# szpajder/dumpvdl2

Hardware: AMD Instinct MI355X
Metric: IQ MS/s demodulated end-to-end (higher is better)
Workload: dtype f32

## Files before the change

dumpvdl2_amd/csrc/debug_hooks.inc:

```

static bool hip_ok(hipError_t e) { return e == hipSuccess; }
template<typename T> static bool dbg_up(const DevBuf<T> &d, const void *src, size_t bytes) { return hip_ok(hipMemcpy(d, src, bytes, hipMemcpyHostToDevice)); }
template<typename T> static bool dbg_up(const DevBuf<T> &d, const void *src) { return dbg_up(d, src, d.bytes()); }
template<typename T> static bool dbg_fill(const DevBuf<T> &d, int v) { return hip_ok(hipMemset(d, v, d.bytes())); }
template<typename T> static bool dbg_down(void *dst, const DevBuf<T> &d, size_t bytes) { return hip_ok(hipMemcpy(dst, d, bytes, hipMemcpyDeviceToHost)); }
template<typename T> static bool dbg_down(void *dst, const DevBuf<T> &d) { return dbg_down(dst, d, d.bytes()); }
static bool dbg_tables(const DevBuf<Tables> &d) { auto tab = std::make_unique<Tables>(); build_tables(*tab); return dbg_up(d, tab.get()); }

template<int K> static int prof_read(const void *symbol, unsigned long long *out, int reset) {
	unsigned long long h[64][K];
	if(hipMemcpyFromSymbol(h, symbol, sizeof h) != hipSuccess) return -3;
	for(int k = 0; k < K; k++) { out[k] = 0; for(int s = 0; s < 64; s++) out[k] += h[s][k]; }
	if(reset) { memset(h, 0, sizeof h); if(hipMemcpyToSymbol(symbol, h, sizeof h) != hipSuccess) return -3; }
	return 0;
}

extern "C" {

int vdl2hip_debug_live_resources(long long out[3]) {
	if(!out) return VDL2HIP_E_INVAL;
	for(int i = 0; i < 3; i++) out[i] = hostmem::g_live[i].load();
	return VDL2HIP_OK;
}

// ... 41 lines not shown
	DevBuf<ScanReq> d_sq, d_rt; DevBuf<uint32_t> d_n;
	if(!hip_ok(d_sq.alloc(count)) || !hip_ok(d_n.alloc(2)) || !hip_ok(d_rt.alloc(kRetryScans))) return VDL2HIP_E_NOMEM;
	uint32_t before[8] = {0}, after[8] = {0};
	const uint32_t nn[2] = { count, 0u };
	Event e0, e1;
	if(!hip_ok(e0.ensure()) || !hip_ok(e1.ensure()) || !dbg_up(d_sq, h.data()) || !dbg_up(d_n, nn) || !dbg_down(before, c->d_refstats, sizeof before)) return VDL2HIP_E_DEVICE;
	RefChan *ref = c->d_ref[(c->feed_no - 1) % kSlots];
	launch_scans(c, c->streams.front, ref, 0xfffeu, d_sq, nullptr, d_n, count, c->k_total, with_retry ? d_rt.get() : nullptr, d_n + 1, e0, e1);
	if(!hip_ok(hipStreamSynchronize(c->streams.front)) || !dbg_down(after, c->d_refstats, sizeof after)) return VDL2HIP_E_DEVICE;
	if(ms) { float t = 0.f; (void)hipEventElapsedTime(&t, e0, e1); *ms = t; }
	return (int)(after[0] - before[0]);
}
int vdl2hip_debug_exact_window(vdl2hip_ctx *c, uint32_t chan, int64_t n_lo, int64_t n_hi) { return vdl2hip_debug_exact_window_many(c, chan, n_lo, n_hi, 1, 0, nullptr); }

int vdl2hip_debug_u8_levels(float out[512]) {
	DevBuf<float> d;
	if(!hip_ok(d.alloc(512))) return VDL2HIP_E_NOMEM;
	hipLaunchKernelGGL(k_u8_level_probe, dim3(1), dim3(256), 0, 0, d);
	return dbg_down(out, d) ? VDL2HIP_OK : VDL2HIP_E_DEVICE;
}

int vdl2hip_debug_s8_levels(float out[512]) {
	DevBuf<float> d;
	if(!hip_ok(d.alloc(512))) return VDL2HIP_E_NOMEM;
	hipLaunchKernelGGL(k_s8_level_probe, dim3(1), dim3(256), 0, 0, d);
	return dbg_down(out, d) ? VDL2HIP_OK : VDL2HIP_E_DEVICE;
}

int vdl2hip_debug_dpp_probe(const float in[64], float out[256]) {
	DevBuf<float> d_in, d_out;
	if(!hip_ok(d_in.alloc(64)) || !hip_ok(d_out.alloc(256))) return VDL2HIP_E_NOMEM;
	if(!dbg_up(d_in, in)) return VDL2HIP_E_DEVICE;
	hipLaunchKernelGGL(k_dpp_probe, dim3(1), dim3(64), 0, 0, (const float *)d_in, d_out);
	return dbg_down(out, d_out) ? VDL2HIP_OK : VDL2HIP_E_DEVICE;
}

int vdl2hip_debug_core_probe(int kind, const void *in, size_t n, void *out) {
	if(kind < 0 || kind >= PROBE_KINDS || !in || !out || n == 0 || n > (size_t)1 << 26) return VDL2HIP_E_INVAL;
	DevBuf<float> d_in, d_out; DevBuf<Tables> d_tab;
	if(!hip_ok(d_in.alloc(n * (size_t)core_probe_in_words(kind))) || !hip_ok(d_out.alloc(n * (size_t)core_probe_out_words(kind))) || !hip_ok(d_tab.alloc(1))) return VDL2HIP_E_NOMEM;
	if(!dbg_tables(d_tab) || !dbg_up(d_in, in) || !dbg_fill(d_out, 0)) return VDL2HIP_E_DEVICE;
	hipLaunchKernelGGL(k_core_probe, dim3((unsigned)((n + 255) / 256)), dim3(256), 0, 0, kind, (const float *)d_in, (uint32_t)n, d_out, (const Tables *)d_tab);
	return hip_ok(hipGetLastError()) && dbg_down(out, d_out) ? VDL2HIP_OK : VDL2HIP_E_DEVICE;
}

int vdl2hip_debug_burst_probe(int kind, const void *in, size_t n, unsigned grid, void *out, const uint32_t *freq, uint32_t nchan, const float *y, uint32_t ring_len,
		uint32_t cap_frames, uint32_t cap_pool, uint32_t guard_frames, uint32_t guard_pool, void *frames, uint8_t *pool, void *ctl, unsigned long long *cnt) {
	if(kind < 0 || kind >= BPROBE_KINDS || !in || n == 0 || n > (size_t)1 << 20 || grid == 0 || grid > 1024) return VDL2HIP_E_INVAL;
	const uint32_t nwaves = grid * (uint32_t)kBurstWaves;
	const bool burst = kind == BPROBE_BURST;
	size_t nin = 0, nout = 0;
	if(kind == BPROBE_WAVE) { nin = n * 64 * 4; nout = n * (size_t)kBProbeWaveOut * 4; }
	else if(kind == BPROBE_RS) {
		nin = n * (size_t)kBProbeRsStride; nout = n * (size_t)kBProbeRsStride + n * 4;
		for(size_t i = 0; i < n; i++) { const uint8_t np = ((const uint8_t *)in)[i * kBProbeRsStride + kRsN]; if(np > kRsPar || (np & 1)) return VDL2HIP_E_INVAL; }
	} else {
		nin = n * sizeof(Burst);
		if(!freq || nchan == 0 || !y || ring_len < 64 || (ring_len & (ring_len - 1)) || ring_len > 1u << 20 || !frames || !pool || !ctl || !cnt) return VDL2HIP_E_INVAL;
		if(cap_frames > 1u << 20 || cap_pool > 1u << 26 || guard_frames > 1u << 16 || guard_pool > 1u << 20 || n * (size_t)ring_len > (size_t)1 << 26) return VDL2HIP_E_INVAL;
		for(size_t i = 0; i < n; i++) {
			const Burst &b = ((const Burst *)in)[i];
			if(b.chan < 0 || (uint32_t)b.chan >= nchan || b.nsym < 1 || b.nsym > kMaxSyms || b.tl_bits == 0 || b.tl_bits > kMaxTl || b.t_first < 0 || b.prev_n < -2) return VDL2HIP_E_INVAL;
		}
	}
	if(!burst && !out) return VDL2HIP_E_INVAL;
	const size_t nfr = (size_t)cap_frames + guard_frames, npool = (size_t)cap_pool + guard_pool;
// ... 393 lines not shown
```

dumpvdl2_amd/csrc/kernels.h:

```cpp
#pragma once
#include <hip/hip_runtime.h>
#include <type_traits>
#include "vdl2_core.h"
#include "design.h"

#ifndef VDL2_K1_UNROLL
#define VDL2_K1_UNROLL 5
#endif

#ifndef VDL2_K1_WAVES_PER_EU
#define VDL2_K1_WAVES_PER_EU 3
#endif

namespace vdl2 {

constexpr int kK1Unroll = VDL2_K1_UNROLL;
typedef float v2f __attribute__((ext_vector_type(2)));
typedef float v4f __attribute__((ext_vector_type(4)));

#ifndef VDL2_REF_PRIO
#define VDL2_REF_PRIO 3
#endif
#ifndef VDL2_K1_PRIO
#define VDL2_K1_PRIO 0
// ... 239 lines not shown
	const int c = (chan + (int)blockIdx.x) % nchan;
	const int64_t off = stride * (int64_t)blockIdx.x;
	ChanView v{ ref->y + (size_t)c * ref->cap, nullptr, nullptr, ref->mask, ref, c, 0xffffu };
	const bool ok = ref_exact_window(v, n_lo + off, n_hi + off, scratch, REF_CANDIDATE);
	if(threadIdx.x == 0) out[blockIdx.x] = ok ? 1 : 0;
}

VDL2_HD bool ref_window_done(const ChanView &v, int64_t n_lo, int64_t n_hi) {
#if VDL2_DEVICE_PASS
	return ref_window_done_dev(v, n_lo, n_hi);
#else
	(void)v; (void)n_lo; (void)n_hi;
	return false;
#endif
}
VDL2_HD __attribute__((always_inline)) bool ref_exact_window(const ChanView &v, int64_t n_lo, int64_t n_hi, void *scratch, int kind) {
#if VDL2_DEVICE_PASS
	(void)scratch;
	return ref_exact_window_dev(v, n_lo, n_hi, kind);
#else
	(void)v; (void)n_lo; (void)n_hi; (void)scratch; (void)kind;
	return false;
#endif
}

struct K1Consts {
	float g0[kMaxOversample], g1[kMaxOversample];
	float P[4], c0, c1, c2, pad_;
	float Q[6][4];
	float Pp[kRunMax + 1][4];
	float cP[kRunMax][2];
};

inline K1Consts make_k1_consts(const BlockForm &bf) {
	K1Consts k{};
	for(int i = 0; i < kMaxOversample; i++) { k.g0[i] = bf.g0[i]; k.g1[i] = bf.g1[i]; }
	for(int i = 0; i < 4; i++) k.P[i] = bf.P[i];
	k.c0 = bf.c0; k.c1 = bf.c1; k.c2 = bf.c2;
	for(int d = 0; d < 6; d++) for(int i = 0; i < 4; i++) k.Q[d][i] = bf.Q[d][i];
	for(int r = 0; r <= kRunMax; r++) for(int i = 0; i < 4; i++) k.Pp[r][i] = bf.Ppow[r][i];
	for(int r = 0; r < kRunMax; r++) { k.cP[r][0] = bf.cP[r][0]; k.cP[r][1] = bf.cP[r][1]; }
	return k;
}

struct K1Args {
	const void *in;
	const void *carry;
	uint32_t ncarry;
	uint64_t nlogical;
	uint64_t n0;
	int64_t  k0;
	int64_t  D;
	int32_t  fmt, nchan, os, nseg, gy;
	int32_t  seg0, seg1;
	const uint32_t *dphi;
	const Lut4 *lut;
	K1Consts bf;
	cf32 *y;
	float4 *seg_end;
	const float4 *qpow;
	int32_t  tiles;
	int32_t  fuse;
	const float4 *carry_in;
	float4 *carry_out;
	const BlockForm *bfd;
	unsigned long long *seg_pub;
	uint32_t epoch;
	uint32_t pub_epoch;
	uint32_t spin_limit;
	uint32_t *sync_timeouts;
	uint32_t cap, mask, nseg_cap;
// ... 27 lines not shown
__device__ __forceinline__ float dpp_row_shr(float v, int d) {
	const int x = __builtin_bit_cast(int, v);
	int r;
	switch(d) {
		case 0: r = __builtin_amdgcn_update_dpp(0, x, 0x111, 0xf, 0xf, true); break;
		case 1: r = __builtin_amdgcn_update_dpp(0, x, 0x112, 0xf, 0xf, true); break;
		case 2: r = __builtin_amdgcn_update_dpp(0, x, 0x114, 0xf, 0xf, true); break;
		default: r = __builtin_amdgcn_update_dpp(0, x, 0x118, 0xf, 0xf, true); break;
	}
	return __builtin_bit_cast(float, r);
}
template<int CTRL, int ROWS>
__device__ __forceinline__ float dpp_bcast(float v) {
	return __builtin_bit_cast(float, __builtin_amdgcn_update_dpp(0, __builtin_bit_cast(int, v), CTRL, ROWS, 0xf, false));
}
template<int CTRL, int ROWS>
__device__ __forceinline__ float dpp_bcast_keep(float old, float v) {
	return __builtin_bit_cast(float, __builtin_amdgcn_update_dpp(__builtin_bit_cast(int, old), __builtin_bit_cast(int, v), CTRL, ROWS, 0xf, false));
}
__device__ __forceinline__ float dpp_wave_shr1_keep(float lane0, float v) {
	return __builtin_bit_cast(float, __builtin_amdgcn_update_dpp(__builtin_bit_cast(int, lane0), __builtin_bit_cast(int, v), 0x138, 0xf, 0xf, false));
}
__device__ __forceinline__ float dpp_wave_shr1(float v) {
	return __builtin_bit_cast(float, __builtin_amdgcn_update_dpp(0, __builtin_bit_cast(int, v), 0x138, 0xf, 0xf, true));
}

__global__ void k_dpp_probe(const float *in, float *out) {
	const int l = threadIdx.x & 63;
	const float v = in[l];
	out[l] = dpp_row_shr(v, 2);
	out[64 + l] = dpp_bcast<0x142, 0xa>(v);
	out[128 + l] = dpp_bcast<0x143, 0xc>(v);
	out[192 + l] = dpp_wave_shr1(v);
}

#ifndef VDL2_K1_MIN_BLOCKS
#define VDL2_K1_MIN_BLOCKS 6
#endif
#ifndef VDL2_K1_MIN_BLOCKS_CR4
#define VDL2_K1_MIN_BLOCKS_CR4 4
#endif
#ifdef VDL2_K1_PROF
__device__ unsigned long long vdl2_k1_prof[64][16];
#define K1_BEGIN() unsigned k1_t0_ = (unsigned)__builtin_readcyclecounter(), k1_acc_[8] = {0, 0, 0, 0, 0, 0, 0, 0}, k1_tiles_ = 0
#define K1_MARK(k) do { if(__builtin_amdgcn_readfirstlane(threadIdx.x >> 6) == 0) { const unsigned t_ = (unsigned)__builtin_readcyclecounter(); \
	k1_acc_[k] += t_ - k1_t0_; if((k) == 3) k1_tiles_++; k1_t0_ = t_; } } while(0)
#define K1_END() do { if(threadIdx.x == 0) { for(int k_ = 0; k_ < 8; k_++) atomicAdd(&vdl2_k1_prof[blockIdx.x & 63][k_], (unsigned long long)k1_acc_[k_]); \
	atomicAdd(&vdl2_k1_prof[blockIdx.x & 63][8], 1ull); atomicAdd(&vdl2_k1_prof[blockIdx.x & 63][9], (unsigned long long)k1_tiles_); } } while(0)
#else
#define K1_BEGIN() do {} while(0)
#define K1_MARK(k) do {} while(0)
#define K1_END() do {} while(0)
#endif

__device__ __forceinline__ float u8_level(uint32_t i) {
	const float d = (float)i - 127.5f, r = 1.0f / 127.5f;
	const float q = d * r;
	return __builtin_fmaf(__builtin_fmaf(-127.5f, q, d), r, q);
}
__global__ void k_u8_level_probe(float *out) { const uint32_t i = threadIdx.x; out[i] = u8_level(i); out[256 + i] = ((float)i - 127.5f) / 127.5f; }
__device__ __forceinline__ float2 s8_level(uint32_t w) {
	const uint32_t u = w ^ 0x8080u;
	return make_float2(__builtin_fmaf((float)(u & 0xffu), 0.0078125f, -1.0f), __builtin_fmaf((float)((u >> 8) & 0xffu), 0.0078125f, -1.0f));
}
__global__ void k_s8_level_probe(float *out) { const uint32_t i = threadIdx.x; out[i] = i & 1 ? s8_level(i << 8).y : s8_level(i).x; out[256 + i] = (float)(int8_t)i / 128.0f; }

// ... 7 lines not shown
	float *o = out + (size_t)i * core_probe_out_words(kind);
	switch(kind) {
	case PROBE_PHASE: o[0] = phase_of(cf32{x[0], x[1]}); break;
	case PROBE_PHASE_FAST: o[0] = phase_fast(cf32{x[0], x[1]}); break;
	case PROBE_MAG: o[0] = mag_of(cf32{x[0], x[1]}); break;
	case PROBE_METRIC: {
		float ph[kPreamble];
		for(int j = 0; j < kPreamble; j++) ph[j] = x[j];
		sync_metric(ph, *tab, o[0], o[1]);
	} break;
	case PROBE_SCREEN: {
		float ph[kPreamble];
		for(int j = 0; j < kPreamble; j++) ph[j] = x[j];
		o[0] = sync_metric_screen(ph, kPreamble); o[1] = sync_metric_screen(ph, kScreenEarly);
	} break;
	case PROBE_SLICE: {
		int neg = 0;
		const int idx = slice_symbol(x[0], x[1], x[2], neg);
		o[0] = __int_as_float(idx); o[1] = __int_as_float(neg);
	} break;
	case PROBE_VERTEX: o[0] = parabola_vertex(x[0], x[1], x[2]); break;
	case PROBE_PPM: {
		const uint32_t freq = __float_as_uint(x[1]);
		o[0] = ppm_of(x[0], freq); o[1] = ppm_gate_threshold(freq, x[2]);
	} break;
	case PROBE_HEADER: {
		const Geometry g = header_to_geometry(__float_as_uint(x[0]), tab->hdr_H, tab->hdr_fix);
		o[0] = __int_as_float(g.status); o[1] = __uint_as_float(g.syndrome); o[2] = __uint_as_float(g.tl_bits); o[3] = __uint_as_float(g.want_bits);
	} break;
	default: break;
	}
}

template<int OS, int R, int CR, bool U8 = false, bool CF32 = false, bool S8 = false>
__global__ __launch_bounds__(256, (CR >= 4 ? VDL2_K1_MIN_BLOCKS_CR4 : VDL2_K1_MIN_BLOCKS)) void k_chanfir(K1Args a) {
	static_assert(64 * R == kFixW || R == 1, "the fused fix-up assumes the fix window is the segment's first tile");
	static_assert(R >= 1 && R <= 2, "the run's outputs are held in two register pairs");
	__shared__ __align__(16) float4 lut[256];
	__shared__ __align__(16) float4 qpow[64];
	__shared__ __align__(16) float park[4 * 4 * 4 * 4];
	__shared__ int fallback;
	constexpr bool kParkY = OS != 0 && CR >= 4 && R == 2;
	__shared__ __align__(8) float2 ypark[kParkY ? CR * 256 : 1];
	extern __shared__ __align__(16) unsigned char smem[];
	if(VDL2_K1_PRIO) __builtin_amdgcn_s_setprio(VDL2_K1_PRIO);
	const int os = OS ? OS : a.os;
	const int run = R * os;
	float2 *tile = (float2 *)smem;
	const int tid = threadIdx.x;
	K1_BEGIN();

	const int bid = blockIdx.x;
	const int xcd = bid & 7, q = bid >> 3;
	const int gy = q % a.gy;
	const int seg = a.seg0 + (q / a.gy) * 8 + xcd;
	if(seg >= a.seg1) return;

	constexpr bool kPrefetch = OS != 0 && CR >= 4 && (64 * R * OS + 255) / 256 <= 10 && (64 * R * OS) % 256 == 0;
	static_assert(!U8 || kPrefetch, "the unsigned-byte build exists where the tile prefetch does");
	static_assert(!CF32 || !U8, "one format per build");
	static_assert(!S8 || (kPrefetch && !U8 && !CF32), "the signed-byte build exists where the unsigned-byte build does, one format per build");
	constexpr bool kByte = U8 || S8;
	constexpr int kFmt = CF32 ? 2 : S8 ? 3 : U8 ? 0 : 1;
	constexpr int kLoadS8 = S8 ? 2 : (kPrefetch && (OS == 20 || OS == 10)) ? 0 : 1;
	constexpr int kPre = kPrefetch ? (64 * R * OS) / 256 : 1;
	constexpr bool kPipeGather = kPrefetch;
	uint32_t pre[kPre]; bool have_pre = false;
	float2 pre2[CF32 ? kPre : 1];
	#pragma unroll
	for(int k = 0; k < kPre; k++) pre[k] = 0u;
	#pragma unroll
	for(int k = 0; k < (CF32 ? kPre : 1); k++) pre2[k] = make_float2(0.f, 0.f);
	if(kPrefetch) {
		const int64_t s0 = (int64_t)seg * a.tiles * (64 * R * (OS ? OS : 1));
		have_pre = a.fmt == kFmt && s0 >= (int64_t)a.ncarry && s0 + 64 * R * (OS ? OS : 1) <= (int64_t)a.nlogical && (int64_t)seg * a.tiles * (64 * R) < a.D;
		if(have_pre) {
			if constexpr(CF32) {
				const float2 *sn = (const float2 *)a.in + (s0 - a.ncarry);
				#pragma unroll
				for(int k = 0; k < kPre; k++) pre2[k] = sn[tid + 256 * k];
			} else if constexpr(kByte) {
				const uint16_t *sn = (const uint16_t *)a.in + (s0 - a.ncarry);
				#pragma unroll
				for(int k = 0; k < kPre; k++) pre[k] = sn[tid + 256 * k];
			} else {
			const uint32_t *sn = (const uint32_t *)a.in + (s0 - a.ncarry);
			#pragma unroll
			for(int k = 0; k < kPre; k++) pre[k] = sn[tid + 256 * k];
			}
		}
	}
	lut[tid] = ((const float4 *)a.lut)[tid];
	if(tid < 64) qpow[tid] = a.qpow[tid];
	if(tid == 0) fallback = 0;
	const int wave = __builtin_amdgcn_readfirstlane(tid >> 6), lane = tid & 63;
	const int cbase = (gy * 4 + wave) * CR;
	const bool wave_active = cbase < a.nchan;
	const K1Consts &bf = a.bf;
	const int tile_n = 64 * run;
	const int L = 64 * R;

	uint32_t dph[CR];
	float4 *carry = (float4 *)(park + wave * (4 * CR * 4));
	float4 *svp = carry + CR;
	float4 *sendp = svp + CR;
	float4 *tsp = sendp + CR;
#ifdef VDL2_K1_HOLD_IN_MEMORY
	constexpr bool kHoldRegs = !(OS != 0 && CR >= 4);
#else
	constexpr bool kHoldRegs = true;
#endif
	float hold[CR][4];
	#pragma unroll
	for(int c = 0; c < CR; c++) hold[c][0] = hold[c][1] = hold[c][2] = hold[c][3] = 0.f;
	#pragma unroll
	for(int c = 0; c < CR; c++) {
		const int ch = cbase + c < a.nchan ? cbase + c : a.nchan - 1;
		dph[c] = a.dphi[ch];
		if(lane == 0) carry[c] = make_float4(0.f, 0.f, 0.f, 0.f);
	}
	const float P0 = bf.P[0], P1 = bf.P[1], P2 = bf.P[2], P3 = bf.P[3];
	const float c0 = bf.c0, c1 = bf.c1, c2 = bf.c2;

	for(int ts = 0; ts < a.tiles; ts++) {
		const int64_t tix = (int64_t)seg * a.tiles + ts;
		const int64_t kbase = tix * L;
		if(kbase >= a.D) break;
		const int64_t sbase = tix * tile_n;
		K1_MARK(ts ? 4 : 0);
		if(ts) __syncthreads();
		K1_MARK(5);
		const bool fast_now = a.fmt == kFmt && sbase >= (int64_t)a.ncarry && sbase + tile_n <= (int64_t)a.nlogical;
		if(CF32 && kPrefetch && fast_now) {
			const float2 *src = (const float2 *)a.in + (sbase - a.ncarry);
			#pragma unroll
			for(int k = 0; k < kPre; k++) {
				const int t = tid + 256 * k;
				const float2 w = have_pre ? pre2[CF32 ? k : 0] : src[t];
				const int l = t / run, m = t - l * run;
				tile[m * 65 + l] = make_float2(cf32_level(w.x), cf32_level(w.y));
			}
			const int64_t snext = sbase + tile_n;
			have_pre = ts + 1 < a.tiles && (tix + 1) * L < a.D && snext + tile_n <= (int64_t)a.nlogical;
			if(have_pre) {
				const float2 *sn = (const float2 *)a.in + (snext - a.ncarry);
				#pragma unroll
				for(int k = 0; k < kPre; k++) pre2[CF32 ? k : 0] = sn[tid + 256 * k];
			}
		} else if(!CF32 && kPrefetch && kByte && fast_now) {
			const uint16_t *src = (const uint16_t *)a.in + (sbase - a.ncarry);
			#pragma unroll
			for(int k = 0; k < kPre; k++) {
				const int t = tid + 256 * k;
				const uint32_t w = have_pre ? pre[k] : (uint32_t)src[t];
				const int l = t / run, m = t - l * run;
				if constexpr(S8) tile[m * 65 + l] = s8_level(w);
				else tile[m * 65 + l] = make_float2(u8_level(w & 0xffu), u8_level((w >> 8) & 0xffu));
			}
			const int64_t snext = sbase + tile_n;
			have_pre = ts + 1 < a.tiles && (tix + 1) * L < a.D && snext + tile_n <= (int64_t)a.nlogical;
			if(have_pre) {
				const uint16_t *sn = (const uint16_t *)a.in + (snext - a.ncarry);
				#pragma unroll
				for(int k = 0; k < kPre; k++) pre[k] = sn[tid + 256 * k];
			}
		} else if(!CF32 && kPrefetch && fast_now) {
// ... 4 lines not shown
			}
			#pragma unroll
			for(int k = 0; k < kPre; k++) {
				const int t = tid + 256 * k;
				const uint32_t w = pre[k];
				const int l = t / run, m = t - l * run;
				tile[m * 65 + l] = make_float2((float)(int16_t)(w & 0xffff) / 32768.0f, (float)(int16_t)(w >> 16) / 32768.0f);
			}
			const int64_t snext = sbase + tile_n;
			have_pre = ts + 1 < a.tiles && (tix + 1) * L < a.D && snext + tile_n <= (int64_t)a.nlogical;
			if(have_pre) {
				const uint32_t *sn = (const uint32_t *)a.in + (snext - a.ncarry);
				#pragma unroll
				for(int k = 0; k < kPre; k++) pre[k] = sn[tid + 256 * k];
			}
		} else if(!CF32 && fast_now) {
			const uint32_t *src = (const uint32_t *)a.in + (sbase - a.ncarry);
			for(int t = tid; t < tile_n; t += 256) {
				const uint32_t w = src[t];
				const int l = t / run, m = t - l * run;
				tile[m * 65 + l] = make_float2((float)(int16_t)(w & 0xffff) / 32768.0f, (float)(int16_t)(w >> 16) / 32768.0f);
			}
		} else {
			int64_t sb = sbase;
			asm volatile("" : "+s"(sb));
			for(int t = tid; t < tile_n; t += 256) {
				const int64_t sidx = sb + t;
				float re = 0.f, im = 0.f;
				if(sidx < (int64_t)a.nlogical) load_sample<CF32, kLoadS8>(a, sidx, re, im);
				const int l = t / run, m = t - l * run;
				tile[m * 65 + l] = make_float2(re, im);
			}
		}
		K1_MARK(1);
		__syncthreads();
		K1_MARK(2);
		if(!wave_active) continue;

		uint32_t ph[CR];
		const uint32_t nabs = (uint32_t)((a.n0 + (uint64_t)sbase + (uint64_t)lane * run) & 0xffffffu);
		#pragma unroll
		for(int c = 0; c < CR; c++) ph[c] = nabs * dph[c];
		const int64_t rem = a.D - kbase;
		const int blast = rem >= L ? L - 1 : (int)rem - 1;
		const int lb = blast / R, ib = blast - lb * R;

		float t0r[CR], t0i[CR], t1r[CR], t1i[CR];
		float ya[CR][2], yb[CR][2];
		#pragma unroll
		for(int c = 0; c < CR; c++) {
			t0r[c] = t0i[c] = t1r[c] = t1i[c] = 0.f;
			ya[c][0] = ya[c][1] = yb[c][0] = yb[c][1] = 0.f;
		}

		#pragma unroll 1
		for(int i = 0; i < R; i++) {
			v2f A0[CR], A1[CR], M[CR];
			#pragma unroll
			for(int c = 0; c < CR; c++) { A0[c] = v2f{0.f, 0.f}; A1[c] = v2f{0.f, 0.f}; M[c] = v2f{0.f, 0.f}; }
			const float2 *trow = tile + (size_t)(i * os) * 65 + lane;
			float4 en = kPipeGather ? lut[(ph[0] >> 16) & 0xffu] : make_float4(0.f, 0.f, 0.f, 0.f);
			#pragma unroll kK1Unroll
			for(int j = 0; j < os; j++) {
				const float2 x = trow[j * 65];
				const v2f X = v2f{x.x, x.y}, Xr = v2f{-x.y, x.x};
				const float g0 = bf.g0[j], g1 = bf.g1[j];
				#pragma unroll
				for(int c = 0; c < CR; c++) {
					const uint32_t p = ph[c];
					const float F = (float)(p & 0xffffu);
					float4 e;
					if(kPipeGather) {
						e = en;
						ph[c] = p + dph[c];
						en = lut[(ph[(c + 1) % CR] >> 16) & 0xffu];
					} else e = lut[(p >> 16) & 0xffu];
					const v2f sc = __builtin_elementwise_fma(v2f{e.z, e.w}, v2f{F, F}, v2f{e.x, e.y});
					const v2f m = __builtin_elementwise_fma(v2f{sc.y, sc.y}, X, v2f{sc.x, sc.x} * Xr);
					A0[c] = __builtin_elementwise_fma(v2f{g0, g0}, m, A0[c]);
					A1[c] = __builtin_elementwise_fma(v2f{g1, g1}, m, A1[c]);
					M[c] = m;
					if(!kPipeGather) ph[c] = p + dph[c];
				}
			}
			float a0r[CR], a0i[CR], a1r[CR], a1i[CR], lr[CR], li[CR];
			#pragma unroll
			for(int c = 0; c < CR; c++) { a0r[c] = A0[c].x; a0i[c] = A0[c].y; a1r[c] = A1[c].x; a1i[c] = A1[c].y; lr[c] = M[c].x; li[c] = M[c].y; }
			#pragma unroll
			for(int c = 0; c < CR; c++) {
				const float n0r = __builtin_fmaf(P0, t0r[c], __builtin_fmaf(P1, t1r[c], a0r[c]));
				const float n0i = __builtin_fmaf(P0, t0i[c], __builtin_fmaf(P1, t1i[c], a0i[c]));
				const float n1r = __builtin_fmaf(P2, t0r[c], __builtin_fmaf(P3, t1r[c], a1r[c]));
				const float n1i = __builtin_fmaf(P2, t0i[c], __builtin_fmaf(P3, t1i[c], a1i[c]));
				t0r[c] = n0r; t0i[c] = n0i; t1r[c] = n1r; t1i[c] = n1i;
				const float yr = __builtin_fmaf(c0, n0r, __builtin_fmaf(c1, n1r, c2 * lr[c]));
				const float yi = __builtin_fmaf(c0, n0i, __builtin_fmaf(c1, n1i, c2 * li[c]));
				if(kParkY) {
					if(i == 0) ypark[c * 256 + tid] = make_float2(yr, yi);
					yb[c][0] = yr; yb[c][1] = yi;
				} else if(i == 0) { ya[c][0] = yr; ya[c][1] = yi; } else { yb[c][0] = yr; yb[c][1] = yi; }
			}
			if(i == ib && lane == lb) {
				#pragma unroll
				for(int c = 0; c < CR; c++) svp[c] = make_float4(t0r[c], t0i[c], t1r[c], t1i[c]);
			}
		}

		K1_MARK(3);
		#pragma unroll
		for(int d = 0; d < 4; d++) {
			const float q0 = bf.Q[d][0], q1 = bf.Q[d][1], q2 = bf.Q[d][2], q3 = bf.Q[d][3];
			#pragma unroll
			for(int c = 0; c < CR; c++) {
				const float o0r = dpp_row_shr(t0r[c], d), o0i = dpp_row_shr(t0i[c], d);
				const float o1r = dpp_row_shr(t1r[c], d), o1i = dpp_row_shr(t1i[c], d);
				t0r[c] = __builtin_fmaf(q0, o0r, __builtin_fmaf(q1, o1r, t0r[c])); t0i[c] = __builtin_fmaf(q0, o0i, __builtin_fmaf(q1, o1i, t0i[c]));
// ... 82 lines not shown
		if(lane == 63) {
			#pragma unroll
			for(int c = 0; c < CR; c++) carry[c] = make_float4(t0r[c], t0i[c], t1r[c], t1i[c]);
		}
	}
	K1_MARK(4);
	if(!a.fuse) { K1_END(); return; }

	bool timed_out = false;
	if(wave_active) {
		if(seg == 0) {
			if(lane < CR) tsp[lane] = a.carry_in[cbase + lane < a.nchan ? cbase + lane : a.nchan - 1];
		} else if(lane < 4 * CR) {
			const int c = lane >> 2, ch = cbase + c < a.nchan ? cbase + c : a.nchan - 1;
			const unsigned long long *src = a.seg_pub + ((size_t)ch * a.nseg_cap + seg - 1) * 4 + (lane & 3);
			unsigned long long w = __hip_atomic_load(src, __ATOMIC_RELAXED, __HIP_MEMORY_SCOPE_AGENT);
			for(int spins = 0; (uint32_t)(w >> 32) != a.epoch; spins++) {
				if((uint32_t)spins > a.spin_limit) { timed_out = true; break; }
				__builtin_amdgcn_s_sleep(8);
				w = __hip_atomic_load(src, __ATOMIC_RELAXED, __HIP_MEMORY_SCOPE_AGENT);
			}
			reinterpret_cast<float *>(tsp)[lane] = __uint_as_float((uint32_t)w);
		}
	}
	if(timed_out) fallback = 1;
	__syncthreads();
	K1_MARK(6);
	if(fallback) {
		if(tid == 0) atomicAdd(a.sync_timeouts, 1u);
		const int64_t sbase = ((int64_t)seg * a.tiles - 1) * tile_n;
		for(int t = tid; t < tile_n; t += 256) {
			const int64_t sidx = sbase + t;
			float re = 0.f, im = 0.f;
			if(sidx >= 0 && sidx < (int64_t)a.nlogical) load_sample<CF32, kLoadS8>(a, sidx, re, im);
			const int l = t / run, m = t - l * run;
			tile[m * 65 + l] = make_float2(re, im);
		}
		__syncthreads();
		if(wave_active) {
			const uint32_t nabs = (uint32_t)((a.n0 + (uint64_t)sbase + (uint64_t)lane * run) & 0xffffffu);
			const float4 qw = lane < 63 ? qpow[62 - lane] : make_float4(1.f, 0.f, 0.f, 1.f);
			#pragma unroll 1
			for(int c = 0; c < CR; c++) {
				uint32_t p = nabs * dph[c];
				float u0r = 0.f, u0i = 0.f, u1r = 0.f, u1i = 0.f;
				#pragma unroll 1
				for(int i = 0; i < R; i++) {
					v2f A0 = v2f{0.f, 0.f}, A1 = v2f{0.f, 0.f};
					const float2 *trow = tile + (size_t)(i * os) * 65 + lane;
					#pragma unroll 1
					for(int j = 0; j < os; j++) {
						const float2 x = trow[j * 65];
						const v2f X = v2f{x.x, x.y}, Xr = v2f{-x.y, x.x};
						const float F = (float)(p & 0xffffu);
						const float4 e = lut[(p >> 16) & 0xffu];
						const v2f sc = __builtin_elementwise_fma(v2f{e.z, e.w}, v2f{F, F}, v2f{e.x, e.y});
						const v2f m = __builtin_elementwise_fma(v2f{sc.y, sc.y}, X, v2f{sc.x, sc.x} * Xr);
						A0 = __builtin_elementwise_fma(v2f{bf.g0[j], bf.g0[j]}, m, A0);
						A1 = __builtin_elementwise_fma(v2f{bf.g1[j], bf.g1[j]}, m, A1);
						p += dph[c];
					}
					const float n0r = __builtin_fmaf(P0, u0r, __builtin_fmaf(P1, u1r, A0.x)), n0i = __builtin_fmaf(P0, u0i, __builtin_fmaf(P1, u1i, A0.y));
					const float n1r = __builtin_fmaf(P2, u0r, __builtin_fmaf(P3, u1r, A1.x)), n1i = __builtin_fmaf(P2, u0i, __builtin_fmaf(P3, u1i, A1.y));
					u0r = n0r; u0i = n0i; u1r = n1r; u1i = n1i;
				}
				float s0r = qw.x * u0r + qw.y * u1r, s0i = qw.x * u0i + qw.y * u1i, s1r = qw.z * u0r + qw.w * u1r, s1i = qw.z * u0i + qw.w * u1i;
				#pragma unroll
				for(int d = 1; d < 64; d <<= 1) { s0r += __shfl_xor(s0r, d); s0i += __shfl_xor(s0i, d); s1r += __shfl_xor(s1r, d); s1i += __shfl_xor(s1i, d); }
				if(lane == 0) tsp[c] = make_float4(s0r, s0i, s1r, s1i);
			}
		}
	}
	if(!wave_active) return;
	__builtin_amdgcn_fence(__ATOMIC_ACQ_REL, "wavefront");
	__builtin_amdgcn_wave_barrier();
	const int64_t seglen = (int64_t)a.tiles * L;
	const int64_t kloc0 = (int64_t)seg * seglen + (int64_t)lane * R;
	#pragma unroll
	for(int c = 0; c < CR; c++) {
		const bool cvalid = cbase + c < a.nchan;
		const float4 ts = tsp[c];
		const int i0 = lane * R;
		float v0r = hold[c][0], v0i = hold[c][1], v1r = hold[c][2], v1i = hold[c][3];
		if(!kHoldRegs) {
			const cf32 *yin = a.y + (size_t)(cbase + c) * a.cap;
// ... 1258 lines not shown
```

dumpvdl2_amd/csrc/vdl2hip.hip:

```cpp
#include <hip/hip_runtime.h>
#include <hip/hip_ext.h>
#include <algorithm>
#include <cmath>
#include <cstddef>
#include <cstdio>
#include <cstdlib>
#include <cstring>
#include <deque>
#include <map>
#include <memory>
#include <mutex>
#include <new>
#include <string>
#include <vector>
#include "../../include/vdl2hip.h"
#include "kernels.h"
#include "resample.h"
#include "resample_design.h"
#include "spectrum.h"
#include "spectrum_design.h"
#include "activity.h"
#include "txlog.h"
#include "capture.h"
#include "tables.h"
// ... 159 lines not shown
	DevBuf<WalkState> d_ws_snap[2], d_ws_tmp; DevBuf<unsigned long long> d_cnt_snap[2], d_cnt_tmp; uint32_t rq_cap = 8192; uint32_t sq_alloc = 8192;
	int walk_ahead = 1; bool walk_ahead_auto = true; double walk_ahead_below = 1.1e8; int debug_force_mismatch = 0; uint32_t debug_mark_cap = 0;
	int ref_retry_mul = 2;
	DevBuf<RefChan> d_ref[kSlots]; DevBuf<unsigned long long> d_refdone; DevBuf<uint32_t> d_refdonen, d_refstats; DevBuf<uint8_t> d_mix;
	std::vector<uint64_t> statsd_prev;
	std::vector<HostFrame> queue;
	int64_t k_total = 0; uint64_t n_total = 0;
	int profiling = 0;
	vdl2hip_stats stats{};
};

#define HIPCHK(expr) do { hipError_t e_ = (expr); if(e_ != hipSuccess) { \
	fprintf(stderr, "vdl2hip: %s failed: %s (%s:%d)\n", #expr, hipGetErrorString(e_), __FILE__, __LINE__); return VDL2HIP_E_DEVICE; } } while(0)

constexpr int kFmtS8 = 3;
static int fmt_code(uint32_t sample_fmt) {
	switch(sample_fmt) {
		case VDL2HIP_FMT_U8: case VDL2HIP_FMT_S16LE: case VDL2HIP_FMT_CF32: return (int)sample_fmt;
		case VDL2HIP_FMT_S8: return kFmtS8;
		default: return -1;
	}
}
static size_t sample_bytes(int fmt) { return fmt == VDL2HIP_FMT_CF32 ? 8 : fmt == VDL2HIP_FMT_S16LE ? 4 : 2; }

struct OnDevice {
	int prev = -1; bool switched = false;
	explicit OnDevice(const vdl2hip_ctx *c) { if(c && hipGetDevice(&prev) == hipSuccess && prev != c->cfg.device) switched = hipSetDevice(c->cfg.device) == hipSuccess; }
	~OnDevice() { if(switched) (void)hipSetDevice(prev); }
};

#define LAUNCH_EV(kernel, grid, block, stream, e0, e1, ...) hipExtLaunchKernelGGL(kernel, grid, block, 0u, stream, e0, e1, 0, __VA_ARGS__)
#define EV(i) (prof_all ? (hipEvent_t)ev[i] : (hipEvent_t) nullptr)

template<int OS, int R>
static void launch_chanfir(vdl2hip_ctx *c, const K1Args &a, int cr, size_t lds, hipEvent_t e0, hipEvent_t e1) {
	const int groups = (c->C + cr - 1) / cr;
	K1Args b = a;
	b.gy = (groups + 3) / 4;
	const int nseg8 = (a.seg1 - a.seg0 + 7) / 8 * 8;
	dim3 grid((unsigned)(nseg8 * b.gy)), block(256);
	if(c->fmt == VDL2HIP_FMT_CF32) {
		switch(cr) {
			case 4: hipExtLaunchKernelGGL((k_chanfir<OS, R, 4, false, true>), grid, block, (uint32_t)lds, c->streams.front, e0, e1, 0, b); break;
			case 2: hipExtLaunchKernelGGL((k_chanfir<OS, R, 2, false, true>), grid, block, (uint32_t)lds, c->streams.front, e0, e1, 0, b); break;
			default: hipExtLaunchKernelGGL((k_chanfir<OS, R, 1, false, true>), grid, block, (uint32_t)lds, c->streams.front, e0, e1, 0, b); break;
		}
		return;
	}
	switch(cr) {
		case 4:
			if constexpr(OS == 20 || OS == 10) { if(c->fmt == VDL2HIP_FMT_U8) { hipExtLaunchKernelGGL((k_chanfir<OS, R, 4, true>), grid, block, (uint32_t)lds, c->streams.front, e0, e1, 0, b); break; } }
			if constexpr(OS == 20 || OS == 10) { if(c->fmt == kFmtS8) { hipExtLaunchKernelGGL((k_chanfir<OS, R, 4, false, false, true>), grid, block, (uint32_t)lds, c->streams.front, e0, e1, 0, b); break; } }
			hipExtLaunchKernelGGL((k_chanfir<OS, R, 4>), grid, block, (uint32_t)lds, c->streams.front, e0, e1, 0, b); break;
		case 2: hipExtLaunchKernelGGL((k_chanfir<OS, R, 2>), grid, block, (uint32_t)lds, c->streams.front, e0, e1, 0, b); break;
		default: hipExtLaunchKernelGGL((k_chanfir<OS, R, 1>), grid, block, (uint32_t)lds, c->streams.front, e0, e1, 0, b); break;
	}
}

static int launch_back(vdl2hip_ctx *c, OutSlot &sl);
static int capture_launch(vdl2hip_ctx *c, OutSlot &sl, hipStream_t st);
static void capture_free(vdl2hip_ctx *c);
static int launch_rest(vdl2hip_ctx *c, OutSlot &sl, struct OutSlot *succ);
static int flush_rest(vdl2hip_ctx *c, const OutSlot *upto);
static bool feed_is_small(const vdl2hip_ctx *c, int64_t D);

static int capture_collect(vdl2hip_ctx *c, OutSlot &sl, const OutFrame *fr, uint32_t nf);
static int txlog_collect(vdl2hip_ctx *c, OutSlot &sl, const OutFrame *fr, uint32_t nf);
static int collect_slot(vdl2hip_ctx *c, OutSlot &sl) {
	if(!sl.pending) return VDL2HIP_OK;
	if(sl.rest_pending) { int r = flush_rest(c, &sl); if(r != VDL2HIP_OK) return r; }
	HIPCHK(hipEventSynchronize(sl.done));
	sl.pending = false;
	sl.rs_t.collect(c->stats.resample_ms);
	sl.mon_t.collect(c->mon.kernel_ms);
	sl.act_t.collect(c->act.kernel_ms);
	sl.cap_t.collect(c->capt.kernel_ms);
	sl.txl_t.collect(c->txl.kernel_ms);
	if(c->profiling && sl.ev_valid) {
		const Event *ev = sl.ev;
		float ms = 0.f;
		if(sl.k1_timed && hipEventElapsedTime(&ms, ev[0], ev[1]) == hipSuccess) { c->stats.chanfir_ms += ms; c->stats.chanfir_launches++; }
		if(sl.ev_level >= 2) {
		if(!sl.fused && hipEventElapsedTime(&ms, ev[2], ev[3]) == hipSuccess) c->stats.phase_ms += ms;
		if(hipEventElapsedTime(&ms, ev[4], sl.ev_front) == hipSuccess) c->stats.sync_ms += ms;
		if(hipEventElapsedTime(&ms, ev[6], ev[7]) == hipSuccess) c->stats.walk_ms += ms;
		if(sl.small) {
// ... 73 lines not shown
	}
	HIPCHK(hipGetLastError());
	if(c->txl.on && nb) { int r = txlog_launch(c, sl, m0, (uint32_t)nb); if(r != VDL2HIP_OK) return r; }
	HIPCHK(m.tap.mark(c->streams.front));
	t.launched(nb ? 2 : 1);
	m.bins = m1; m.carry_sel ^= 1;
	return VDL2HIP_OK;
}
static void activity_free(vdl2hip_ctx *c) {
	auto &m = c->act;
	if(m.tap.queued) (void)hipEventSynchronize(m.tap.last);
	m.buf = {};
	m.on = false; m.tap.queued = false;
}

static int feed_common(vdl2hip_ctx *c, const void *dev_in, size_t nbytes, bool in_parts = false) {
	const size_t sb = sample_bytes(c->fmt);
	const uint64_t nnew = nbytes / sb;
	const uint64_t nlogical = c->ncarry + nnew;
	const int64_t D = (int64_t)(nlogical / (uint64_t)c->os);
	const uint32_t nrem = (uint32_t)(nlogical - (uint64_t)D * c->os);
	const int seglen = 64 * c->run;
	if(c->failed) return VDL2HIP_E_DEVICE;
	OutSlot &sl = c->slot[c->feed_no % kSlots];
	{ int r = collect_slot(c, sl); if(r != VDL2HIP_OK && r != VDL2HIP_E_OVERFLOW) return r; }
	hipStream_t st = c->streams.front;
	const Event *ev = sl.ev;
	const bool prof = c->profiling != 0, prof_all = c->profiling >= 2;

	K1Args a{};
	a.in = dev_in; a.carry = c->d_carry[c->carry_sel]; a.ncarry = c->ncarry; a.nlogical = nlogical;
	a.n0 = c->n_total - c->ncarry; a.k0 = c->k_total; a.D = D;
	a.fmt = c->fmt; a.nchan = c->C; a.os = c->os; a.nseg = 0; a.gy = 1;
	a.dphi = c->d_dphi; a.lut = c->d_lut; a.bf = make_k1_consts(c->bf); a.y = c->d_y; a.seg_end = c->d_segend;
	a.qpow = c->d_qpow; a.cap = c->cap; a.mask = c->cap - 1; a.nseg_cap = c->nseg_cap;
	a.fuse = c->fuse_k2 && 64 * c->run == kFixW; a.carry_in = c->d_tcarry[c->tcarry_sel]; a.carry_out = c->d_tcarry[c->tcarry_sel ^ 1];
	a.bfd = c->d_bf; a.seg_pub = c->d_segpub; a.epoch = (uint32_t)(c->feed_no + 1); a.sync_timeouts = c->d_synctmo;
	a.pub_epoch = a.epoch; a.spin_limit = 4096;
	if(c->debug_force_timeout) { a.pub_epoch = a.epoch ^ 0x40000000u; a.spin_limit = 16; }
	{
		const int64_t ntile = (D + seglen - 1) / seglen;
		const int groups = (c->C + c->cr - 1) / c->cr, gy = (groups + 3) / 4;
		int64_t tiles = ntile * gy / 6144; if(tiles < 1) tiles = 1; if(tiles > 8) tiles = 8;
		a.tiles = (int)tiles;
		a.nseg = (int)((ntile + tiles - 1) / tiles);
	}

	sl.ev_valid = false;
	sl.cap_on = c->capt.on && D > 0;
	sl.txl_on = false;
	if(D > 0) {
		const size_t lds = (size_t)c->run * c->os * 65 * sizeof(float2);
		const bool cold = in_parts && c->cold.n > 1;
		if(cold) c->stats.cold_start_feeds++;
		sl.k1_timed = prof && !cold;
		hipEvent_t e0 = sl.k1_timed ? (hipEvent_t)ev[0] : nullptr, e1 = sl.k1_timed ? (hipEvent_t)ev[1] : nullptr;
		auto launch = [&](int seg0, int seg1, hipEvent_t s_ev, hipEvent_t p_ev) {
			a.seg0 = seg0; a.seg1 = seg1;
			if(c->specialised) {
				switch(c->os) {
					case 20: launch_chanfir<20, kRun>(c, a, c->cr, lds, s_ev, p_ev); break;
					case 13: launch_chanfir<13, kRun>(c, a, c->cr, lds, s_ev, p_ev); break;
					default: launch_chanfir<10, kRun>(c, a, c->cr, lds, s_ev, p_ev); break;
				}
			} else {
				launch_chanfir<0, kRunGeneric>(c, a, c->cr, lds, s_ev, p_ev);
			}
		};
		if(!in_parts || c->cold.n <= 1) launch(0, a.nseg, e0, e1);
		else {
			const uint64_t seg_in = (uint64_t)a.tiles * (uint64_t)seglen * (uint64_t)c->os;
			int done = 0;
			for(int p = 0; p < c->cold.n; p++) {
				HIPCHK(hipStreamWaitEvent(st, c->cold.ev[p], 0));
				int ready = a.nseg;
				if(p < c->cold.n - 1) { const uint64_t r = (c->ncarry + c->cold.samples[p]) / seg_in; ready = r >= (uint64_t)a.nseg ? a.nseg : (int)(r & ~7ull); }
				if(ready > done) { launch(done, ready, done == 0 ? e0 : (hipEvent_t) nullptr, ready == a.nseg ? e1 : (hipEvent_t) nullptr); done = ready; }
			}
		}
		if(!a.fuse) {
			K2Args k2{ c->d_y, c->d_segend, c->d_tcarry[c->tcarry_sel], c->d_tcarry[c->tcarry_sel ^ 1], c->d_bf,
			           c->k_total, D, c->cap, c->cap - 1, c->nseg_cap, seglen * a.tiles };
			LAUNCH_EV(k_fixup, dim3((unsigned)((D + 255) / 256), (unsigned)c->C), dim3(256), st, EV(2), EV(3), k2);
		}
		c->tcarry_sel ^= 1;
// ... 1403 lines not shown
```

Baseline: 5627.

## Stage raw cs16 tiles into LDS via async global-to-LDS DMA with double buffering

For the cs16 format with oversample 20 or 10 and four channels per block, the channel FIR kernel now copies raw packed int16 samples straight into LDS with global_load_lds_dwordx4. It uses two tile buffers so the next tile's copy overlaps the current tile's compute, and drops one of the two block barriers per tile. Samples are converted to float inside the inner loop, and the 1/32768 scale is folded into the filter constants. A packed multiply with operand select replaces building the rotated sample vector. The raw tile uses less LDS than the float2 tile, which could raise occupancy. The cost is hand-written inline assembly that saves and restores m0, plus extra int-to-float conversions in the hot loop.

```diff
diff --git a/dumpvdl2_amd/csrc/debug_hooks.inc b/dumpvdl2_amd/csrc/debug_hooks.inc
--- a/dumpvdl2_amd/csrc/debug_hooks.inc
+++ b/dumpvdl2_amd/csrc/debug_hooks.inc
@@ -97,6 +97,15 @@
 	if(!hip_ok(d_in.alloc(64)) || !hip_ok(d_out.alloc(256))) return VDL2HIP_E_NOMEM;
 	if(!dbg_up(d_in, in)) return VDL2HIP_E_DEVICE;
 	hipLaunchKernelGGL(k_dpp_probe, dim3(1), dim3(64), 0, 0, (const float *)d_in, d_out);
+	return dbg_down(out, d_out) ? VDL2HIP_OK : VDL2HIP_E_DEVICE;
+}
+
+int vdl2hip_debug_glds_probe(const uint32_t *in, uint32_t n, uint32_t off, uint32_t out[2560]) {
+	if(!in || !out || n < 2560 || off > n - 2560) return VDL2HIP_E_INVAL;
+	DevBuf<uint32_t> d_in, d_out;
+	if(!hip_ok(d_in.alloc(n)) || !hip_ok(d_out.alloc(2560))) return VDL2HIP_E_NOMEM;
+	if(!dbg_up(d_in, in)) return VDL2HIP_E_DEVICE;
+	hipLaunchKernelGGL(k_glds_probe, dim3(1), dim3(256), 0, 0, (const uint32_t *)d_in, off, (uint32_t *)d_out);
 	return dbg_down(out, d_out) ? VDL2HIP_OK : VDL2HIP_E_DEVICE;
 }
 
diff --git a/dumpvdl2_amd/csrc/kernels.h b/dumpvdl2_amd/csrc/kernels.h
--- a/dumpvdl2_amd/csrc/kernels.h
+++ b/dumpvdl2_amd/csrc/kernels.h
@@ -295,11 +295,12 @@
 	float cP[kRunMax][2];
 };
 
-inline K1Consts make_k1_consts(const BlockForm &bf) {
+inline K1Consts make_k1_consts(const BlockForm &bf, bool raw = false) {
 	K1Consts k{};
-	for(int i = 0; i < kMaxOversample; i++) { k.g0[i] = bf.g0[i]; k.g1[i] = bf.g1[i]; }
+	const float s = raw ? 1.0f / 32768.0f : 1.0f;
+	for(int i = 0; i < kMaxOversample; i++) { k.g0[i] = bf.g0[i] * s; k.g1[i] = bf.g1[i] * s; }
 	for(int i = 0; i < 4; i++) k.P[i] = bf.P[i];
-	k.c0 = bf.c0; k.c1 = bf.c1; k.c2 = bf.c2;
+	k.c0 = bf.c0; k.c1 = bf.c1; k.c2 = bf.c2 * s;
 	for(int d = 0; d < 6; d++) for(int i = 0; i < 4; i++) k.Q[d][i] = bf.Q[d][i];
 	for(int r = 0; r <= kRunMax; r++) for(int i = 0; i < 4; i++) k.Pp[r][i] = bf.Ppow[r][i];
 	for(int r = 0; r < kRunMax; r++) { k.cP[r][0] = bf.cP[r][0]; k.cP[r][1] = bf.cP[r][1]; }
@@ -393,6 +394,43 @@
 	out[64 + l] = dpp_bcast<0x142, 0xa>(v);
 	out[128 + l] = dpp_bcast<0x143, 0xc>(v);
 	out[192 + l] = dpp_wave_shr1(v);
+}
+
+__device__ __forceinline__ void glds16(const void *gbase, uint32_t voff, uint32_t lds_dst) {
+	uint32_t keep;
+	asm volatile("s_mov_b32 %0, m0\n\ts_mov_b32 m0, %2\n\ts_nop 0\n\tglobal_load_lds_dwordx4 %1, %3\n\ts_mov_b32 m0, %0"
+		: "=&s"(keep) : "v"(voff), "s"(lds_dst), "s"(gbase) : "memory");
+}
+template<int RUN>
+__device__ __forceinline__ void raw_tile_dma(const uint32_t *src, uint32_t lds_dst, int wave, int lane) {
+	static_assert(RUN % 4 == 0, "a group is four samples");
+	constexpr int G = RUN / 4;
+	const uint32_t voff = (uint32_t)lane * (RUN * 4);
+	#pragma unroll
+	for(int k = 0; k < (G + 3) / 4; k++) {
+		const int g = wave + 4 * k;
+		if(g < G) glds16(src + 4 * g, voff, lds_dst + (uint32_t)g * 1024u);
+	}
+}
+__device__ __forceinline__ v2f mul_sin_ix(v2f sc, v2f x) {
+	v2f r;
+	asm("v_pk_mul_f32 %0, %1, %2 op_sel:[1,0] op_sel_hi:[0,0] neg_lo:[1,0]" : "=v"(r) : "v"(x), "v"(sc));
+	return r;
+}
+__device__ __forceinline__ int raw_tile_word(int l, int m) { return (m >> 2) * 256 + l * 4 + (m & 3); }
+__device__ __forceinline__ void raw_tile_barrier() { asm volatile("s_waitcnt vmcnt(0) lgkmcnt(0)\n\ts_barrier" ::: "memory"); }
+__device__ __forceinline__ uint32_t lds_address(const void *p) {
+	return (uint32_t)__builtin_amdgcn_readfirstlane((int)(uintptr_t)(const __attribute__((address_space(3))) void *)p);
+}
+
+__global__ __launch_bounds__(256) void k_glds_probe(const uint32_t *in, uint32_t off, uint32_t *out) {
+	__shared__ __align__(16) uint32_t t[40 * 64];
+	const int tid = threadIdx.x;
+	for(int k = tid; k < 40 * 64; k += 256) t[k] = 0xdeadbeefu;
+	raw_tile_barrier();
+	raw_tile_dma<40>(in + off, lds_address(t), __builtin_amdgcn_readfirstlane(tid >> 6), tid & 63);
+	raw_tile_barrier();
+	for(int k = tid; k < 40 * 64; k += 256) out[k] = t[k];
 }
 
 #ifndef VDL2_K1_MIN_BLOCKS
@@ -466,7 +504,7 @@
 	}
 }
 
-template<int OS, int R, int CR, bool U8 = false, bool CF32 = false, bool S8 = false>
+template<int OS, int R, int CR, bool U8 = false, bool CF32 = false, bool S8 = false, bool RAW = false>
 __global__ __launch_bounds__(256, (CR >= 4 ? VDL2_K1_MIN_BLOCKS_CR4 : VDL2_K1_MIN_BLOCKS)) void k_chanfir(K1Args a) {
 	static_assert(64 * R == kFixW || R == 1, "the fused fix-up assumes the fix window is the segment's first tile");
 	static_assert(R >= 1 && R <= 2, "the run's outputs are held in two register pairs");
@@ -481,6 +519,7 @@
 	const int os = OS ? OS : a.os;
 	const int run = R * os;
 	float2 *tile = (float2 *)smem;
+	uint32_t *rawt = (uint32_t *)smem;
 	const int tid = threadIdx.x;
 	K1_BEGIN();
 
@@ -497,7 +536,10 @@
 	constexpr bool kByte = U8 || S8;
 	constexpr int kFmt = CF32 ? 2 : S8 ? 3 : U8 ? 0 : 1;
 	constexpr int kLoadS8 = S8 ? 2 : (kPrefetch && (OS == 20 || OS == 10)) ? 0 : 1;
-	constexpr int kPre = kPrefetch ? (64 * R * OS) / 256 : 1;
+	static_assert(!RAW || (kPrefetch && !U8 && !CF32 && !S8 && (R * OS) % 4 == 0), "the raw tile is the cs16 prefetch builds'");
+	constexpr int kPre = kPrefetch && !RAW ? (64 * R * OS) / 256 : 1;
+	constexpr int kRawWords = RAW ? 64 * R * OS : 0;
+	const uint32_t raw_lds = RAW ? lds_address(smem) : 0u;
 	constexpr bool kPipeGather = kPrefetch;
 	uint32_t pre[kPre]; bool have_pre = false;
 	float2 pre2[CF32 ? kPre : 1];
@@ -508,7 +550,9 @@
 	if(kPrefetch) {
 		const int64_t s0 = (int64_t)seg * a.tiles * (64 * R * (OS ? OS : 1));
 		have_pre = a.fmt == kFmt && s0 >= (int64_t)a.ncarry && s0 + 64 * R * (OS ? OS : 1) <= (int64_t)a.nlogical && (int64_t)seg * a.tiles * (64 * R) < a.D;
-		if(have_pre) {
+		if constexpr(RAW) {
+			if(have_pre) raw_tile_dma<R * OS>((const uint32_t *)a.in + (s0 - a.ncarry), raw_lds, __builtin_amdgcn_readfirstlane(tid >> 6), tid & 63);
+		} else if(have_pre) {
 			if constexpr(CF32) {
 				const float2 *sn = (const float2 *)a.in + (s0 - a.ncarry);
 				#pragma unroll
@@ -562,10 +606,29 @@
 		if(kbase >= a.D) break;
 		const int64_t sbase = tix * tile_n;
 		K1_MARK(ts ? 4 : 0);
-		if(ts) __syncthreads();
+		if(!RAW && ts) __syncthreads();
 		K1_MARK(5);
 		const bool fast_now = a.fmt == kFmt && sbase >= (int64_t)a.ncarry && sbase + tile_n <= (int64_t)a.nlogical;
-		if(CF32 && kPrefetch && fast_now) {
+		if constexpr(RAW) {
+			if(!have_pre) {
+				int64_t sb = sbase;
+				asm volatile("" : "+s"(sb));
+				uint32_t *dst = rawt + (ts & 1) * kRawWords;
+				for(int t = tid; t < tile_n; t += 256) {
+					const int64_t sidx = sb + t;
+					uint32_t w = 0u;
+					if(sidx < (int64_t)a.nlogical) w = sidx < (int64_t)a.ncarry ? ((const uint32_t *)a.carry)[sidx] : ((const uint32_t *)a.in)[sidx - a.ncarry];
+					const int l = t / run;
+					dst[raw_tile_word(l, t - l * run)] = w;
+				}
+			}
+			K1_MARK(1);
+			raw_tile_barrier();
+			K1_MARK(2);
+			const int64_t snext = sbase + tile_n;
+			have_pre = ts + 1 < a.tiles && (tix + 1) * L < a.D && snext >= (int64_t)a.ncarry && snext + tile_n <= (int64_t)a.nlogical;
+			if(have_pre) raw_tile_dma<R * OS>((const uint32_t *)a.in + (snext - a.ncarry), raw_lds + (uint32_t)(((ts + 1) & 1) * kRawWords * 4), wave, lane);
+		} else if(CF32 && kPrefetch && fast_now) {
 			const float2 *src = (const float2 *)a.in + (sbase - a.ncarry);
 			#pragma unroll
 			for(int k = 0; k < kPre; k++) {
@@ -636,9 +699,11 @@
 				tile[m * 65 + l] = make_float2(re, im);
 			}
 		}
+		if constexpr(!RAW) {
 		K1_MARK(1);
 		__syncthreads();
 		K1_MARK(2);
+		}
 		if(!wave_active) continue;
 
 		uint32_t ph[CR];
@@ -664,11 +729,7 @@
 			for(int c = 0; c < CR; c++) { A0[c] = v2f{0.f, 0.f}; A1[c] = v2f{0.f, 0.f}; M[c] = v2f{0.f, 0.f}; }
 			const float2 *trow = tile + (size_t)(i * os) * 65 + lane;
 			float4 en = kPipeGather ? lut[(ph[0] >> 16) & 0xffu] : make_float4(0.f, 0.f, 0.f, 0.f);
-			#pragma unroll kK1Unroll
-			for(int j = 0; j < os; j++) {
-				const float2 x = trow[j * 65];
-				const v2f X = v2f{x.x, x.y}, Xr = v2f{-x.y, x.x};
-				const float g0 = bf.g0[j], g1 = bf.g1[j];
+			auto sample = [&](const v2f X, const v2f Xr, const float g0, const float g1) __attribute__((always_inline)) {
 				#pragma unroll
 				for(int c = 0; c < CR; c++) {
 					const uint32_t p = ph[c];
@@ -680,12 +741,37 @@
 						en = lut[(ph[(c + 1) % CR] >> 16) & 0xffu];
 					} else e = lut[(p >> 16) & 0xffu];
 					const v2f sc = __builtin_elementwise_fma(v2f{e.z, e.w}, v2f{F, F}, v2f{e.x, e.y});
-					const v2f m = __builtin_elementwise_fma(v2f{sc.y, sc.y}, X, v2f{sc.x, sc.x} * Xr);
+					v2f sx;
+					if constexpr(RAW) sx = mul_sin_ix(sc, X);
+					else sx = v2f{sc.x, sc.x} * Xr;
+					const v2f m = __builtin_elementwise_fma(v2f{sc.y, sc.y}, X, sx);
 					A0[c] = __builtin_elementwise_fma(v2f{g0, g0}, m, A0[c]);
 					A1[c] = __builtin_elementwise_fma(v2f{g1, g1}, m, A1[c]);
 					M[c] = m;
 					if(!kPipeGather) ph[c] = p + dph[c];
 				}
+			};
+			if constexpr(RAW) {
+				constexpr int GW = OS % 4 == 0 ? 4 : 2;
+				const uint32_t *rrow = rawt + (ts & 1) * kRawWords + lane * 4;
+				#pragma unroll 1
+				for(int jj = 0; jj < OS / GW; jj++) {
+					const int m0 = i * OS + jj * GW;
+					uint32_t w[4] = {0u, 0u, 0u, 0u};
+					if constexpr(GW == 4) { const uint4 q = *(const uint4 *)(rrow + (m0 >> 2) * 256); w[0] = q.x; w[1] = q.y; w[2] = q.z; w[3] = q.w; }
+					else { const uint2 q = *(const uint2 *)(rrow + (m0 >> 2) * 256 + (m0 & 3)); w[0] = q.x; w[1] = q.y; }
+					#pragma unroll
+					for(int k = 0; k < GW; k++) {
+						const v2f X = v2f{(float)(int16_t)(w[k] & 0xffffu), (float)(int16_t)(w[k] >> 16)};
+						sample(X, X, bf.g0[jj * GW + k], bf.g1[jj * GW + k]);
+					}
+				}
+			} else {
+			#pragma unroll kK1Unroll
+			for(int j = 0; j < os; j++) {
+				const float2 x = trow[j * 65];
+				sample(v2f{x.x, x.y}, v2f{-x.y, x.x}, bf.g0[j], bf.g1[j]);
+			}
 			}
 			float a0r[CR], a0i[CR], a1r[CR], a1i[CR], lr[CR], li[CR];
 			#pragma unroll
@@ -834,8 +920,14 @@
 		for(int t = tid; t < tile_n; t += 256) {
 			const int64_t sidx = sbase + t;
 			float re = 0.f, im = 0.f;
+			const int l = t / run, m = t - l * run;
+			if constexpr(RAW) {
+				uint32_t w = 0u;
+				if(sidx >= 0 && sidx < (int64_t)a.nlogical) w = sidx < (int64_t)a.ncarry ? ((const uint32_t *)a.carry)[sidx] : ((const uint32_t *)a.in)[sidx - a.ncarry];
+				rawt[raw_tile_word(l, m)] = w;
+				continue;
+			}
 			if(sidx >= 0 && sidx < (int64_t)a.nlogical) load_sample<CF32, kLoadS8>(a, sidx, re, im);
-			const int l = t / run, m = t - l * run;
 			tile[m * 65 + l] = make_float2(re, im);
 		}
 		__syncthreads();
@@ -852,7 +944,9 @@
 					const float2 *trow = tile + (size_t)(i * os) * 65 + lane;
 					#pragma unroll 1
 					for(int j = 0; j < os; j++) {
-						const float2 x = trow[j * 65];
+						float2 x;
+						if constexpr(RAW) { const uint32_t w = rawt[raw_tile_word(lane, i * os + j)]; x = make_float2((float)(int16_t)(w & 0xffffu), (float)(int16_t)(w >> 16)); }
+						else x = trow[j * 65];
 						const v2f X = v2f{x.x, x.y}, Xr = v2f{-x.y, x.x};
 						const float F = (float)(p & 0xffffu);
 						const float4 e = lut[(p >> 16) & 0xffu];
diff --git a/dumpvdl2_amd/csrc/vdl2hip.hip b/dumpvdl2_amd/csrc/vdl2hip.hip
--- a/dumpvdl2_amd/csrc/vdl2hip.hip
+++ b/dumpvdl2_amd/csrc/vdl2hip.hip
@@ -215,6 +215,8 @@
 #define LAUNCH_EV(kernel, grid, block, stream, e0, e1, ...) hipExtLaunchKernelGGL(kernel, grid, block, 0u, stream, e0, e1, 0, __VA_ARGS__)
 #define EV(i) (prof_all ? (hipEvent_t)ev[i] : (hipEvent_t) nullptr)
 
+static bool k1_raw_tile(const vdl2hip_ctx *c) { return c->specialised && (c->os == 20 || c->os == 10) && c->cr == 4 && c->fmt == VDL2HIP_FMT_S16LE; }
+
 template<int OS, int R>
 static void launch_chanfir(vdl2hip_ctx *c, const K1Args &a, int cr, size_t lds, hipEvent_t e0, hipEvent_t e1) {
 	const int groups = (c->C + cr - 1) / cr;
@@ -234,7 +236,9 @@
 		case 4:
 			if constexpr(OS == 20 || OS == 10) { if(c->fmt == VDL2HIP_FMT_U8) { hipExtLaunchKernelGGL((k_chanfir<OS, R, 4, true>), grid, block, (uint32_t)lds, c->streams.front, e0, e1, 0, b); break; } }
 			if constexpr(OS == 20 || OS == 10) { if(c->fmt == kFmtS8) { hipExtLaunchKernelGGL((k_chanfir<OS, R, 4, false, false, true>), grid, block, (uint32_t)lds, c->streams.front, e0, e1, 0, b); break; } }
-			hipExtLaunchKernelGGL((k_chanfir<OS, R, 4>), grid, block, (uint32_t)lds, c->streams.front, e0, e1, 0, b); break;
+			if constexpr(OS == 20 || OS == 10) hipExtLaunchKernelGGL((k_chanfir<OS, R, 4, false, false, false, true>), grid, block, (uint32_t)lds, c->streams.front, e0, e1, 0, b);
+			else hipExtLaunchKernelGGL((k_chanfir<OS, R, 4>), grid, block, (uint32_t)lds, c->streams.front, e0, e1, 0, b);
+			break;
 		case 2: hipExtLaunchKernelGGL((k_chanfir<OS, R, 2>), grid, block, (uint32_t)lds, c->streams.front, e0, e1, 0, b); break;
 		default: hipExtLaunchKernelGGL((k_chanfir<OS, R, 1>), grid, block, (uint32_t)lds, c->streams.front, e0, e1, 0, b); break;
 	}
@@ -374,7 +378,7 @@
 	a.in = dev_in; a.carry = c->d_carry[c->carry_sel]; a.ncarry = c->ncarry; a.nlogical = nlogical;
 	a.n0 = c->n_total - c->ncarry; a.k0 = c->k_total; a.D = D;
 	a.fmt = c->fmt; a.nchan = c->C; a.os = c->os; a.nseg = 0; a.gy = 1;
-	a.dphi = c->d_dphi; a.lut = c->d_lut; a.bf = make_k1_consts(c->bf); a.y = c->d_y; a.seg_end = c->d_segend;
+	a.dphi = c->d_dphi; a.lut = c->d_lut; a.bf = make_k1_consts(c->bf, k1_raw_tile(c)); a.y = c->d_y; a.seg_end = c->d_segend;
 	a.qpow = c->d_qpow; a.cap = c->cap; a.mask = c->cap - 1; a.nseg_cap = c->nseg_cap;
 	a.fuse = c->fuse_k2 && 64 * c->run == kFixW; a.carry_in = c->d_tcarry[c->tcarry_sel]; a.carry_out = c->d_tcarry[c->tcarry_sel ^ 1];
 	a.bfd = c->d_bf; a.seg_pub = c->d_segpub; a.epoch = (uint32_t)(c->feed_no + 1); a.sync_timeouts = c->d_synctmo;
@@ -392,7 +396,7 @@
 	sl.cap_on = c->capt.on && D > 0;
 	sl.txl_on = false;
 	if(D > 0) {
-		const size_t lds = (size_t)c->run * c->os * 65 * sizeof(float2);
+		const size_t lds = k1_raw_tile(c) ? 2 * (size_t)c->run * c->os * 64 * sizeof(uint32_t) : (size_t)c->run * c->os * 65 * sizeof(float2);
 		const bool cold = in_parts && c->cold.n > 1;
 		if(cold) c->stats.cold_start_feeds++;
 		sl.k1_timed = prof && !cold;
```

New measurement: 5620 (median of 4 runs). About the same (-0.1%).
